# CloudEngineHub/FairyGen

Hardware: AMD Instinct MI355X
Metric: decoded frames/sec (sec/clip in config), Wan2.2-TI2V-5B 704x1280x121 @ 5 steps (higher is better)
Workload: dtype bf16

## Files before the change

fairygen_amd/csrc/attention.hip:

```cpp
#include "common.h"
#include <math.h>
#include <queue>
#include <type_traits>
#include <vector>

#include "attn_w4_asm.inc"
#include "attn_w4p_asm.inc"
#ifndef FG_ATTN_W4
#define FG_ATTN_W4 1
#endif

namespace {

constexpr int kD = 128;
constexpr int kBN = 64;
constexpr int kTileBytes = kBN * kD * 2;
constexpr float kDeferLog2 = 6.0f;

typedef __attribute__((address_space(3))) s16x4 lds_s16x4;

__device__ __forceinline__ int k_lds_off(int row, int chunk) { return row * 256 + ((chunk ^ (row & 15)) << 4); }
__device__ __forceinline__ int v_lds_off(int row, int chunk) {
    return 2048 * (row >> 3) + 512 * (chunk >> 2) + 64 * (row & 7) + 16 * ((chunk & 3) ^ ((row >> 2) & 3));
}

__device__ __forceinline__ float fast_exp2(float x) { return __builtin_amdgcn_exp2f(x); }
__device__ __forceinline__ float max3(float a, float b, float c) {
    float r;
    asm("v_max3_f32 %0, %1, %2, %3" : "=v"(r) : "v"(a), "v"(b), "v"(c));
    return r;
}

__device__ __forceinline__ uint32_t cvt_pk_bf16(float lo, float hi) {
    uint32_t r;
    asm("v_cvt_pk_bf16_f32 %0, %1, %2" : "=v"(r) : "v"(lo), "v"(hi));
    return r;
}

template <int I, int N, typename F>
__device__ __forceinline__ void static_for(F&& f) {
    if constexpr (I < N) {
        f(std::integral_constant<int, I>{});
        static_for<I + 1, N>(f);
    }
}
#ifndef FG_EXP_QK
#define FG_EXP_QK 21
#endif
#ifndef FG_KDIST
#define FG_KDIST 3
#endif
#ifndef FG_VDIST
#define FG_VDIST 2
#endif
__host__ __device__ constexpr int exps_before(int g) {
    return g < 16 ? (FG_EXP_QK * g) / 16 : (FG_EXP_QK + (g - 16) < 32 ? FG_EXP_QK + (g - 16) : 32);
}
static_assert(exps_before(27) == 32, "the last exponential must be issued by gap 26 (its pack feeds the MFMA of gap 28)");

__device__ __forceinline__ float add_f32(float a, float b) {
    float r;
    asm("v_add_f32 %0, %1, %2" : "=v"(r) : "v"(a), "v"(b));
    return r;
}

__device__ __forceinline__ float pair_max(float x) {
    auto r = __builtin_amdgcn_permlane32_swap(__float_as_uint(x), __float_as_uint(x), false, false);
    return fmaxf(__uint_as_float(r[0]), __uint_as_float(r[1]));
}
__device__ __forceinline__ float pair_sum(float x) {
    auto r = __builtin_amdgcn_permlane32_swap(__float_as_uint(x), __float_as_uint(x), false, false);
    return __uint_as_float(r[0]) + __uint_as_float(r[1]);
}

#ifndef FG_ATTN_SCHED
#define FG_ATTN_SCHED 1
#endif
#ifndef FG_ATTN_VARIANT
#define FG_ATTN_VARIANT 8
#endif
#if FG_ATTN_VARIANT == 4
constexpr int kBM = 128;
#else
constexpr int kBM = 256;
#endif

struct AttnParams {
    const bf16* q; const bf16* k; const bf16* v; bf16* out;
    int64_t ldq, ldk, ldv, Nq, Nkv;
    int H, nqb, nfull, R, S, total_direct;
    float scale_log2e;
    float* o_part;
    float* ml_part;
};

template <int WAVES, int QB, bool SHORT_KV = false>
__global__ __launch_bounds__(WAVES * 64, QB == 1 ? 2 : 1) void attn_fwd_kernel(const AttnParams P) {
    const bf16* __restrict__ q = P.q; const bf16* __restrict__ k = P.k; const bf16* __restrict__ v = P.v;
    bf16* __restrict__ out = P.out;
    const int64_t ldq = P.ldq, ldk = P.ldk, ldv = P.ldv, Nq = P.Nq, Nkv = P.Nkv;
    const int H = P.H;
    const float scale_log2e = P.scale_log2e;
    static_assert(WAVES * QB * 32 == kBM, "workgroup rows");
    constexpr int THREADS = WAVES * 64;
    constexpr int NST = (kBN * 16) / THREADS;
    constexpr int ST_ROWS = THREADS / 16;
    __shared__ __attribute__((aligned(16))) char smem[4 * kTileBytes];
    char* const k_lds = smem;
    char* const v_lds = smem + 2 * kTileBytes;

    const int nt = (int)((Nkv + kBN - 1) / kBN);
    int qb, bh, t_begin = 0, t_end = nt, piece = -1;
    if ((int)blockIdx.x < P.total_direct) {
        const int bid = blockIdx.x, xcd = bid & 7, slot = bid >> 3;
        const int qd = P.total_direct >> 3, rm = P.total_direct & 7;
        const int logical = (xcd < rm ? xcd * (qd + 1) : rm * (qd + 1) + (xcd - rm) * qd) + slot;
        qb = logical % P.nfull;
        bh = logical / P.nfull;
    } else {
        piece = (int)blockIdx.x - P.total_direct;
        const int sp = piece % P.S, rq = (piece / P.S) % P.R;
        bh = piece / (P.S * P.R);
        qb = P.nfull + rq;
        t_begin = (int)((int64_t)sp * nt / P.S);
        t_end = (int)((int64_t)(sp + 1) * nt / P.S);
    }
    const int b = bh / H, h = bh % H;

    const int tid = threadIdx.x, lane = tid & 63, wave = tid >> 6;
    const int r = lane & 31, hh = lane >> 5;

    const bf16* qp = q + (int64_t)b * Nq * ldq + (int64_t)h * kD;
    const bf16* kp = k + (int64_t)b * Nkv * ldk + (int64_t)h * kD;
    const bf16* vp = v + (int64_t)b * Nkv * ldv + (int64_t)h * kD;
    bf16* op = out + (int64_t)b * Nq * ((int64_t)H * kD) + (int64_t)h * kD;

    int64_t my_q[QB];
    bool q_valid[QB];
    bf16x8 qf[QB][8];
#pragma unroll
    for (int qi = 0; qi < QB; ++qi) {
        my_q[qi] = (int64_t)qb * kBM + (wave * QB + qi) * 32 + r;
        q_valid[qi] = my_q[qi] < Nq;
        if (!q_valid[qi]) my_q[qi] = Nq - 1;
#pragma unroll
        for (int ks = 0; ks < 8; ++ks)
            qf[qi][ks] = *reinterpret_cast<const bf16x8*>(qp + my_q[qi] * ldq + ks * 16 + hh * 8);
    }

    const int st_row = tid >> 4, st_chunk = tid & 15;
    int st_k[NST], st_v[NST];
#pragma unroll
    for (int i = 0; i < NST; ++i) {
        st_k[i] = k_lds_off(st_row + ST_ROWS * i, st_chunk);
// ... 160 lines not shown
        });
        l_run[0] += ps0 + ps1;
        if (!kTail) {
            absorb_max(pair_max(fmaxf(mt, sn[0][1][15])));
        } else if (t + 1 < t_end) {
            if ((int64_t)(t + 2) * kBN > Nkv) mask_tile(sn, t + 1);
            absorb_max(tile_max(sn));
        }
        __syncthreads();
    };

    f32x16 sA[QB][2], sB[QB][2];
    load_k(t_begin);
    load_v(t_begin);
    write_k(0);
    write_v(0);
    load_k(t_begin + 1);
    write_k(1);
    __syncthreads();
    qk_tile(sA, 0);
    if ((int64_t)(t_begin + 1) * kBN > Nkv) mask_tile(sA, t_begin);
    m_run[0] = tile_max(sA);
    __syncthreads();

    const int t_fast = min(t_end - 1, (int)(Nkv / kBN) - 1);
    int t = t_begin;
    for (; t + 1 < t_fast; t += 2) {
        step_sched(sA, sB, t, std::false_type{}, std::integral_constant<int, 0>{});
        step_sched(sB, sA, t + 1, std::false_type{}, std::integral_constant<int, 1>{});
    }
    for (; t < t_end; ++t) {
        step_sched(sA, sB, t, std::true_type{}, std::integral_constant<int, -1>{});
#pragma unroll
        for (int sub = 0; sub < 2; ++sub) sA[0][sub] = sB[0][sub];
    }
#else
    auto step = [&](f32x16 (&sc)[QB][2], f32x16 (&sn)[QB][2], int t) {
        const int cur = (t - t_begin) & 1;
        load_k(t + 2);
        load_v(t + 1);

        qk_tile(sn, cur ^ 1);
        bf16x8 pf[QB][4];
#pragma unroll
        for (int qi = 0; qi < QB; ++qi) {
            float mt = max3(sc[qi][0][0], sc[qi][1][0], sc[qi][0][1]);
            mt = max3(mt, sc[qi][1][1], sc[qi][0][2]);
#pragma unroll
            for (int j = 2; j < 15; ++j) mt = max3(mt, sc[qi][1][j], sc[qi][0][j + 1]);
            mt = pair_max(fmaxf(mt, sc[qi][1][15]));
            const bool grow = (mt - m_run[qi]) * scale_log2e > kDeferLog2;
            if (__builtin_amdgcn_ballot_w64(grow) != 0) {
                const float m_new = fmaxf(m_run[qi], mt);
                const float alpha = fast_exp2((m_run[qi] - m_new) * scale_log2e);
                m_run[qi] = m_new;
                l_run[qi] *= alpha;
#pragma unroll
                for (int i = 0; i < 4; ++i)
#pragma unroll
                    for (int j = 0; j < 16; ++j) o[qi][i][j] *= alpha;
            }
            const float mb = m_run[qi] * scale_log2e;
            float psum = 0.f;
#pragma unroll
            for (int sub = 0; sub < 2; ++sub)
#pragma unroll
                for (int j = 0; j < 16; ++j) {
                    const float p = fast_exp2(sc[qi][sub][j] * scale_log2e - mb);
                    psum += p;
                    pf[qi][sub * 2 + (j >> 3)][j & 7] = (bf16)p;
                }
            l_run[qi] += psum;
        }

        const char* vb = v_lds + cur * kTileBytes;
#pragma unroll
        for (int kk = 0; kk < 4; ++kk) {
#pragma unroll
            for (int db = 0; db < 4; ++db) {
                union { s16x4 h2[2]; bf16x8 f; } a;
                a.h2[0] = __builtin_amdgcn_ds_read_tr16_b64_v4i16((lds_s16x4*)(vb + v_rd0 + 4096 * kk + 512 * db));
                a.h2[1] = __builtin_amdgcn_ds_read_tr16_b64_v4i16((lds_s16x4*)(vb + v_rd1 + 4096 * kk + 512 * db));
#pragma unroll
                for (int qi = 0; qi < QB; ++qi)
                    o[qi][db] = __builtin_amdgcn_mfma_f32_32x32x16_bf16(a.f, pf[qi][kk], o[qi][db], 0, 0, 0);
            }
        }

        write_k(cur);
        write_v(cur ^ 1);
        if ((int64_t)(t + 2) * kBN > Nkv && t + 1 < t_end) mask_tile(sn, t + 1);
        __syncthreads();
    };

    f32x16 sA[QB][2], sB[QB][2];
    load_k(t_begin);
    load_v(t_begin);
    write_k(0);
    write_v(0);
    load_k(t_begin + 1);
    write_k(1);
    __syncthreads();
    qk_tile(sA, 0);
    if ((int64_t)(t_begin + 1) * kBN > Nkv) mask_tile(sA, t_begin);
    __syncthreads();

    int t = t_begin;
    for (; t + 1 < t_end; t += 2) {
        step(sA, sB, t);
        step(sB, sA, t + 1);
    }
    if (t < t_end) step(sA, sB, t);

#endif

#pragma unroll
    for (int qi = 0; qi < QB; ++qi) {
        const float l_tot = pair_sum(l_run[qi]);
        if (piece < 0) {
            const float inv = 1.0f / l_tot;
            if (q_valid[qi]) {
                bf16* orow = op + my_q[qi] * ((int64_t)H * kD);
#pragma unroll
                for (int db = 0; db < 4; ++db)
#pragma unroll
                    for (int g = 0; g < 4; ++g) {
                        bf16x4 w4;
#pragma unroll
                        for (int j = 0; j < 4; ++j) w4[j] = (bf16)(o[qi][db][4 * g + j] * inv);
                        *reinterpret_cast<bf16x4*>(orow + 32 * db + 8 * g + 4 * hh) = w4;
                    }
            }
        } else {
            const int row = (wave * QB + qi) * 32 + r;
            float* orow = P.o_part + ((int64_t)piece * kBM + row) * kD;
#pragma unroll
            for (int db = 0; db < 4; ++db)
#pragma unroll
                for (int g = 0; g < 4; ++g) {
                    f32x4 w4;
#pragma unroll
                    for (int j = 0; j < 4; ++j) w4[j] = o[qi][db][4 * g + j];
                    *reinterpret_cast<f32x4*>(orow + 32 * db + 8 * g + 4 * hh) = w4;
                }
            if (hh == 0) {
                float* ml = P.ml_part + ((int64_t)piece * kBM + row) * 2;
                ml[0] = m_run[qi];
                ml[1] = l_tot;
            }
        }
    }
}

template <bool PRESCALE>
__global__ __launch_bounds__(256, 1) void attn_fwd_w4_kernel(const AttnParams P) {
    const int nt = (int)((P.Nkv + kBN - 1) / kBN);
    int qb, bh, t_begin = 0, t_end = nt, piece = -1;
    if ((int)blockIdx.x < P.total_direct) {
        const int bid = blockIdx.x, xcd = bid & 7, slot = bid >> 3;
        const int qd = P.total_direct >> 3, rm = P.total_direct & 7;
        const int logical = (xcd < rm ? xcd * (qd + 1) : rm * (qd + 1) + (xcd - rm) * qd) + slot;
        qb = logical % P.nfull;
        bh = logical / P.nfull;
    } else {
        piece = (int)blockIdx.x - P.total_direct;
        const int sp = piece % P.S, rq = (piece / P.S) % P.R;
        bh = piece / (P.S * P.R);
        qb = P.nfull + rq;
        t_begin = (int)((int64_t)sp * nt / P.S);
        t_end = (int)((int64_t)(sp + 1) * nt / P.S);
    }
    const int b = bh / P.H, h = bh % P.H;
    const int64_t hd = (int64_t)P.H * kD;
    const bf16* qp = P.q + (int64_t)b * P.Nq * P.ldq + (int64_t)h * kD;
    const bf16* kp = P.k + (int64_t)b * P.Nkv * P.ldk + (int64_t)h * kD;
    const bf16* vp = P.v + (int64_t)b * P.Nkv * P.ldv + (int64_t)h * kD;
    const void* op;
    const void* mlp;
    if (piece < 0) {
        op = P.out + (int64_t)b * P.Nq * hd + (int64_t)h * kD;
        mlp = op;
    } else {
        op = P.o_part + (int64_t)piece * kBM * kD;
        mlp = P.ml_part + (int64_t)piece * kBM * 2;
    }
    auto sgpr = [](uint32_t x) { return (uint32_t)__builtin_amdgcn_readfirstlane(x); };
    auto sptr = [&](const void* p) {
        const uint64_t u = (uint64_t)p;
        return (const void*)(((uint64_t)sgpr((uint32_t)(u >> 32)) << 32) | sgpr((uint32_t)u));
    };
#define FG_ATTN_W4_OPERANDS                                                                                                       \
    "s"(sptr(qp)), "s"(sptr(kp)), "s"(sptr(vp)), "s"(sptr(op)), "s"(sptr(mlp)), "s"(sgpr(threadIdx.x >> 6)),                     \
        "s"(sgpr((uint32_t)t_begin)), "s"(sgpr((uint32_t)t_end)), "s"(sgpr((uint32_t)qb * kBM)), "s"(sgpr(piece < 0 ? 0u : 1u)), \
        "s"(__builtin_amdgcn_kernarg_segment_ptr())
    if constexpr (PRESCALE) asm volatile(FG_ATTN_W4P_ASM : : FG_ATTN_W4_OPERANDS : FG_ATTN_W4P_CLOBBERS);
    else asm volatile(FG_ATTN_W4_ASM : : FG_ATTN_W4_OPERANDS : FG_ATTN_W4_CLOBBERS);
#undef FG_ATTN_W4_OPERANDS
}

static float pow2_scale_log2e(float scale) {
    const double sl = (double)scale * 1.4426950408889634;
    int e = 0;
    const double m = frexp(sl, &e);
    const double p = fabs(m - 0.5) < 0.25 ? ldexp(0.5, e) : ldexp(1.0, e);
    return fabs(sl / p - 1.0) < 1e-6 && e > -100 && e < 100 ? (float)p : 0.f;
}

__global__ __launch_bounds__(256) void attn_combine_kernel(const AttnParams P) {
    const int rows_per_blk = 8, groups = kBM / rows_per_blk;
    const int blk = blockIdx.x / groups, rowgrp = blockIdx.x % groups;
    const int rq = blk % P.R, bh = blk / P.R;
    const int b = bh / P.H, h = bh % P.H;
    const int qb = P.nfull + rq;
    const int lane32 = threadIdx.x & 31, row = rowgrp * rows_per_blk + (threadIdx.x >> 5);
    const int64_t piece0 = ((int64_t)bh * P.R + rq) * P.S;
    const int64_t qrow = (int64_t)qb * kBM + row;
    if (qrow >= P.Nq) return;
    float mmax = -INFINITY;
    for (int sp = 0; sp < P.S; ++sp) mmax = fmaxf(mmax, P.ml_part[((piece0 + sp) * kBM + row) * 2]);
    float denom = 0.f;
    f32x4 acc = {0.f, 0.f, 0.f, 0.f};
    for (int sp = 0; sp < P.S; ++sp) {
        const float* ml = P.ml_part + ((piece0 + sp) * kBM + row) * 2;
        const float w = fast_exp2((ml[0] - mmax) * P.scale_log2e);
        denom += w * ml[1];
        const f32x4 ov = *reinterpret_cast<const f32x4*>(P.o_part + ((piece0 + sp) * kBM + row) * kD + lane32 * 4);
#pragma unroll
        for (int j = 0; j < 4; ++j) acc[j] += w * ov[j];
    }
    const float inv = 1.0f / denom;
    bf16x4 w4;
#pragma unroll
    for (int j = 0; j < 4; ++j) w4[j] = (bf16)(acc[j] * inv);
    *reinterpret_cast<bf16x4*>(P.out + ((int64_t)b * P.Nq + qrow) * ((int64_t)P.H * kD) + (int64_t)h * kD + lane32 * 4) = w4;
}

struct SplitChoice { int R, S; int64_t ws_bytes; double makespan; };

static double simulate_makespan(int64_t n_direct, int64_t n_pieces, double piece_cost, int cus) {
    const int64_t full = n_direct / cus, rem = n_direct % cus;
    if (n_pieces == 0) return (double)(full + (rem ? 1 : 0));
    std::priority_queue<double, std::vector<double>, std::greater<double>> free_at;
    for (int i = 0; i < cus; ++i) free_at.push((double)(full + (i < rem ? 1 : 0)));
    double last = (double)(full + (rem ? 1 : 0));
    for (int64_t i = 0; i < n_pieces; ++i) {
        const double t = free_at.top() + piece_cost;
        free_at.pop();
        free_at.push(t);
        last = t > last ? t : last;
    }
    return last;
}

static SplitChoice choose_split_uncached(int B, int64_t Nq, int64_t Nkv, int H, int cus, int64_t ws_limit) {
    const int64_t nqb = (Nq + kBM - 1) / kBM, bh = (int64_t)B * H;
    const int nt = (int)((Nkv + kBN - 1) / kBN);
    const int64_t per_piece = (int64_t)kBM * kD * 4 + (int64_t)kBM * 2 * 4;
    SplitChoice best{0, 1, 0, simulate_makespan(bh * nqb, 0, 0.0, cus)};
    const double base = best.makespan;
    const int s_list[] = {2, 3, 4, 5, 6, 8, 12, 16};
    for (int mode = 0; mode < 2; ++mode) {
        const int64_t R = mode == 0 ? 1 : nqb;
        if (mode == 0 && nqb < 2) continue;
        if (mode == 1 && bh * nqb > 4 * (int64_t)cus) continue;
        for (int S : s_list) {
            if (S * 8 > nt) break;
            const int64_t pieces = bh * R * S;
            const int64_t ws = pieces * per_piece;
            if (ws > ws_limit) continue;
            const double cost = 1.0 / S + 3.0 / nt + 0.004;
            const double ms = simulate_makespan(bh * (nqb - R), pieces, cost, cus);
            if (ms < best.makespan) best = SplitChoice{(int)R, S, ws, ms};
        }
    }
    if (best.makespan > 0.98 * base) best = SplitChoice{0, 1, 0, base};
    return best;
}

static SplitChoice choose_split(int B, int64_t Nq, int64_t Nkv, int H, int cus, int64_t ws_limit) {
    struct Key { int B, H, cus; int64_t Nq, Nkv, ws; SplitChoice val; };
    static thread_local Key memo[8];
    static thread_local int next = 0, filled = 0;
    for (int i = 0; i < filled; ++i) {
        const Key& e = memo[i];
        if (e.B == B && e.H == H && e.cus == cus && e.Nq == Nq && e.Nkv == Nkv && e.ws == ws_limit) return e.val;
    }
    const SplitChoice val = choose_split_uncached(B, Nq, Nkv, H, cus, ws_limit);
    memo[next] = Key{B, H, cus, Nq, Nkv, ws_limit, val};
    next = (next + 1) % 8;
    if (filled < 8) ++filled;
    return val;
}

static int device_cus() {
    static thread_local int cached_dev = -1, cached_cus = 256;
    int dev = 0;
    if (hipGetDevice(&dev) != hipSuccess) return 256;
    if (dev != cached_dev) {
        int n = 0;
        if (hipDeviceGetAttribute(&n, hipDeviceAttributeMultiprocessorCount, dev) == hipSuccess && n > 0) cached_cus = n;
        cached_dev = dev;
    }
    return cached_cus * (256 / kBM);
}

}

extern "C" int64_t fg_attn_workspace_bytes(int B, int64_t Nq, int64_t Nkv, int H) {
    if (B <= 0 || Nq <= 0 || Nkv <= 0 || H <= 0) return 0;
    return choose_split(B, Nq, Nkv, H, device_cus(), (int64_t)1 << 40).ws_bytes;
}

extern "C" int fg_attn_split_choice(int B, int64_t Nq, int64_t Nkv, int H, int64_t workspace_bytes, int* R, int* S) {
    FG_CHECK_ARG(B > 0 && Nq > 0 && Nkv > 0 && H > 0 && R && S, "fg_attn_split_choice: bad arguments");
    const SplitChoice sc = choose_split(B, Nq, Nkv, H, device_cus(), workspace_bytes);
    *R = sc.R;
    *S = sc.S;
    return FG_OK;
}

extern "C" int fg_attn_fwd_bf16(const void* q, int64_t ldq, const void* k, int64_t ldk, const void* v, int64_t ldv,
                                void* out, int B, int64_t Nq, int64_t Nkv, int H, int D, float scale, void* workspace,
                                int64_t workspace_bytes, fg_stream_t stream) {
    FG_CHECK_ARG(q && k && v && out, "fg_attn_fwd_bf16: null pointer");
    FG_CHECK_ARG(D == kD, "fg_attn_fwd_bf16: only head_dim 128 is supported (got %d)", D);
    FG_CHECK_ARG(B > 0 && H > 0 && Nq > 0 && Nkv > 0, "fg_attn_fwd_bf16: B, H, Nq, Nkv must be positive");
    FG_CHECK_ARG(scale > 0.f, "fg_attn_fwd_bf16: scale must be positive");
    const int64_t hd = (int64_t)H * D;
    FG_CHECK_ARG(ldq >= hd && ldk >= hd && ldv >= hd && ldq % 8 == 0 && ldk % 8 == 0 && ldv % 8 == 0,
                 "fg_attn_fwd_bf16: leading dimensions must be >= H*D and multiples of 8");
    FG_CHECK_ARG(FG_ALIGNED16(q) && FG_ALIGNED16(k) && FG_ALIGNED16(v) && FG_ALIGNED16(out) && FG_ALIGNED16(workspace),
                 "fg_attn_fwd_bf16: pointers must be 16-byte aligned");
    FG_CHECK_ARG(workspace_bytes >= 0 && (workspace != nullptr || workspace_bytes == 0), "fg_attn_fwd_bf16: bad workspace");
    const int64_t nqb = (Nq + kBM - 1) / kBM;
    FG_CHECK_ARG((Nkv + 6 * kBN) * ldk * 2 < (1ll << 32) && (Nkv + 6 * kBN) * ldv * 2 < (1ll << 32),
                 "fg_attn_fwd_bf16: K/V of one batch element must span < 4 GiB (32-bit buffer offsets)");
    FG_CHECK_ARG(Nq * ldq * 2 < (1ll << 32) && Nq * hd * 2 < (1ll << 32),
                 "fg_attn_fwd_bf16: Q / O of one batch element must span < 4 GiB (32-bit buffer offsets)");
    const SplitChoice sc = choose_split(B, Nq, Nkv, H, device_cus(), workspace_bytes);
    AttnParams P;
    P.q = (const bf16*)q; P.k = (const bf16*)k; P.v = (const bf16*)v; P.out = (bf16*)out;
    P.ldq = ldq; P.ldk = ldk; P.ldv = ldv; P.Nq = Nq; P.Nkv = Nkv; P.H = H;
    P.nqb = (int)nqb; P.R = sc.R; P.S = sc.S; P.nfull = (int)(nqb - sc.R);
    const int64_t total_direct = (int64_t)B * H * P.nfull, pieces = (int64_t)B * H * sc.R * sc.S;
    FG_CHECK_ARG(total_direct + pieces < (1ll << 30), "fg_attn_fwd_bf16: grid too large");
    P.total_direct = (int)total_direct;
    P.scale_log2e = scale * 1.4426950408889634f;
    P.o_part = (float*)workspace;
    P.ml_part = (float*)workspace + pieces * kBM * kD;
#if FG_ATTN_VARIANT == 4
    hipLaunchKernelGGL((attn_fwd_kernel<4, 1>), dim3((unsigned)(total_direct + pieces)), dim3(256), 0, (hipStream_t)stream, P);
#else
#if FG_ATTN_W4
    static const bool use_w4 = [] { const char* e = getenv("FAIRYGEN_ATTN_W4"); return e ? atoi(e) != 0 : true; }();
    if (Nkv > 1024 && use_w4) {
        static const hipError_t attr0 = hipFuncSetAttribute(reinterpret_cast<const void*>(attn_fwd_w4_kernel<false>),
                                                            hipFuncAttributeMaxDynamicSharedMemorySize, 8 * kTileBytes);
        static const hipError_t attr1 = hipFuncSetAttribute(reinterpret_cast<const void*>(attn_fwd_w4_kernel<true>),
                                                            hipFuncAttributeMaxDynamicSharedMemorySize, 8 * kTileBytes);
        FG_CHECK_ARG(attr0 == hipSuccess && attr1 == hipSuccess, "fg_attn_fwd_bf16: cannot reserve 128 KiB of LDS: %s",
                     hipGetErrorString(attr0 == hipSuccess ? attr1 : attr0));
        const float p2 = pow2_scale_log2e(scale);
        if (p2 > 0.f) {
            P.scale_log2e = p2;
            hipLaunchKernelGGL(attn_fwd_w4_kernel<true>, dim3((unsigned)(total_direct + pieces)), dim3(256), 8 * kTileBytes, (hipStream_t)stream, P);
        } else {
            hipLaunchKernelGGL(attn_fwd_w4_kernel<false>, dim3((unsigned)(total_direct + pieces)), dim3(256), 8 * kTileBytes, (hipStream_t)stream, P);
        }
    } else
#endif
    if (Nkv <= 1024)
        hipLaunchKernelGGL((attn_fwd_kernel<8, 1, true>), dim3((unsigned)(total_direct + pieces)), dim3(512), 0, (hipStream_t)stream, P);
    else
        hipLaunchKernelGGL((attn_fwd_kernel<8, 1, false>), dim3((unsigned)(total_direct + pieces)), dim3(512), 0, (hipStream_t)stream, P);
#endif
    if (int e = fg_launch_status("fg_attn_fwd_bf16")) return e;
    if (pieces > 0) {
        hipLaunchKernelGGL(attn_combine_kernel, dim3((unsigned)((int64_t)B * H * sc.R * (kBM / 8))), dim3(256), 0, (hipStream_t)stream, P);
        return fg_launch_status("fg_attn_fwd_bf16 (combine)");
    }
    return FG_OK;
}
```

fairygen_amd/hip.py:

```python
import ctypes
import os

import torch

_LIB_PATH = os.environ.get("FAIRYGEN_HIP_LIB") or os.path.join(os.path.dirname(os.path.abspath(__file__)), "libfairygen_hip.so")
_lib = None

ABI_VERSION = 5

_i64, _i32, _f32, _vp = ctypes.c_int64, ctypes.c_int, ctypes.c_float, ctypes.c_void_p

_SIGNATURES = {
    "fg_ln_modulate_bf16": [_vp, _vp, _vp, _vp, _i64, _i32, _f32, _i64, _i64, _i64, _vp],
    "fg_ln_affine_bf16": [_vp, _vp, _vp, _vp, _i64, _i32, _f32, _vp],
    "fg_ln_modulate_fp8_bf16": [_vp, _vp, _vp, _vp, _vp, _i64, _i32, _f32, _i64, _i64, _i64, _f32, _vp],
    "fg_residual_ln_fp8_bf16": [_vp, _vp, _vp, _vp, _vp, _vp, _vp, _vp, _i32, _i64, _i32, _f32, _i64, _i64, _i64, _f32, _vp],
    "fg_ln_modulate_dual_bf16": [_vp, _vp, _vp, _vp, _vp, _vp, _i64, _i32, _f32, _i64, _i64, _i64, _f32, _vp],
    "fg_ln_affine_dual_bf16": [_vp, _vp, _vp, _vp, _vp, _vp, _i64, _i32, _f32, _f32, _vp],
    "fg_gate_residual_bf16": [_vp, _vp, _vp, _vp, _i64, _i32, _i64, _i64, _i64, _vp],
    "fg_residual_ln_bf16": [_vp, _vp, _vp, _vp, _vp, _vp, _vp, _i32, _i64, _i32, _f32, _i64, _i64, _i64, _vp],
    "fg_rmsnorm_rope_bf16": [_vp, _i64, _vp, _vp, _vp, _i32, _vp, _i64, _i32, _i32, _f32, _vp],
    "fg_rmsnorm_rope_grouped_bf16": [_vp, _i64, _vp, _vp, _vp, _i32, _vp, _i64, _i32, _i32, _f32, _i32, _i64, _i64, _vp],
    "fg_copy_groups_bf16": [_vp, _i64, _i64, _vp, _i64, _i64, _i32, _i64, _i32, _vp],
    "fg_fp8_quant_rows_bf16": [_vp, _i64, _vp, _vp, _vp, _i64, _i32, _i32, _f32, _vp],
    "fg_act_bf16": [_vp, _vp, _i64, _i32, _vp],
    "fg_gemm_epilogue_bf16": [_vp, _i64, _vp, _vp, _vp, _i64, _i64, _i64, _i64, _i32, _vp, _i64, _i64, _i64, _vp, _vp],
    "fg_gemm_fp8_bf16": [_vp, _i64, _vp, _vp, _vp, _vp, _i64, _i64, _i64, _i64, _i32, _vp, _i64, _i64, _i64, _vp, _vp],
    "fg_lora_apply_bf16": [_vp, _i64, _vp, _vp, _vp, _i64, _i64, _i64, _i64, _i64, _i64, _i32, _vp, _i64, _i64, _i64, _vp],
    "fg_attn_fwd_bf16": [_vp, _i64, _vp, _i64, _vp, _i64, _vp, _i32, _i64, _i64, _i32, _i32, _f32, _vp, _i64, _vp],
    "fg_cfg_euler_bf16": [_vp, _vp, _vp, _vp, _i64, _f32, _f32, _vp],
    "fg_vae_rmsnorm_silu_bf16": [_vp, _vp, _vp, _i64, _i32, _i32, _vp],
    "fg_conv_pack_weight_bf16": [_vp, _vp, _i32, _i32, _i32, _i32, _i32, _vp],
    "fg_conv3d_cl_bf16": [_vp, _vp, _vp, _vp, _vp, _i32, _i32, _i32, _i32, _i32, _i32, _i32, _i32, _i32, _vp],
    "fg_dupup3d_add_bf16": [_vp, _vp, _vp, _i32, _i32, _i32, _i32, _i32, _i32, _i32, _i32, _vp],
    "fg_softmax_rows_f32_bf16": [_vp, _vp, _i64, _i64, _f32, _vp],
    "fg_vae_latent_to_cl_bf16": [_vp, _vp, _vp, _vp, _i32, _i32, _i32, _i32, _vp],
    "fg_vae_unpatchify_bf16": [_vp, _vp, _i32, _i32, _i32, _i32, _i32, _i32, _vp],
    "fg_vae_tile_accumulate_bf16": [_vp, _vp, _vp, _i32, _i32, _i32, _i32, _i32, _i32, _i32, _i32, _i32, _i32, _i32, _vp],
    "fg_vae_tile_finalize_bf16": [_vp, _vp, _i32, _i32, _i32, _i32, _i32, _vp],
    "fg_vae_patchify_bf16": [_vp, _vp, _i32, _i32, _i32, _vp],
    "fg_avgdown3d_add_bf16": [_vp, _vp, _vp, _i32, _i32, _i32, _i32, _i32, _i32, _i32, _vp],
    "fg_vae_latent_from_cl_bf16": [_vp, _vp, _vp, _vp, _i32, _i32, _i32, _i32, _i32, _vp],
    "fg_video_to_uint8": [_vp, _vp, _i32, _i32, _i32, _vp],
    "fg_softmax_bias_bf16": [_vp, _vp, _vp, _vp, _i64, _i64, _vp],
    "fg_gated_gelu_bf16": [_vp, _vp, _vp, _i64, _vp],
}
EXPORTED_SYMBOLS = sorted(list(_SIGNATURES) + ["fg_version", "fg_last_error", "fg_conv_packed_bytes", "fg_attn_workspace_bytes", "fg_attn_split_choice",
                                                   "fg_conv_tile_choice", "fg_gemm_workspace_bytes", "fg_gemm_debug_grid"])


class HipLibraryError(RuntimeError):
    pass


def library_path():
    return _LIB_PATH


def load():
    global _lib
    if _lib is not None:
        return _lib
    if not os.path.exists(_LIB_PATH):
        raise HipLibraryError(
            f"{_LIB_PATH} not found: build it with `make -C fairygen_amd/csrc` (or __graft_entry__.build()). "
            "fairygen_amd has no CPU / PyTorch fallback for its kernels.")
    lib = ctypes.CDLL(_LIB_PATH)
    lib.fg_version.restype = ctypes.c_int
    lib.fg_last_error.restype = ctypes.c_char_p
    lib.fg_conv_packed_bytes.restype = ctypes.c_int64
    lib.fg_conv_packed_bytes.argtypes = [_i32] * 5
    lib.fg_attn_workspace_bytes.restype = ctypes.c_int64
    lib.fg_attn_workspace_bytes.argtypes = [_i32, _i64, _i64, _i32]
    lib.fg_conv_tile_choice.restype = ctypes.c_int
    lib.fg_conv_tile_choice.argtypes = [_i32] * 4
    lib.fg_gemm_workspace_bytes.restype = ctypes.c_int64
    lib.fg_gemm_workspace_bytes.argtypes = [_i64] * 3
    lib.fg_gemm_debug_grid.restype = ctypes.c_int
    lib.fg_gemm_debug_grid.argtypes = [_i32]
    lib.fg_attn_split_choice.restype = ctypes.c_int
    lib.fg_attn_split_choice.argtypes = [_i32, _i64, _i64, _i32, _i64, ctypes.POINTER(ctypes.c_int), ctypes.POINTER(ctypes.c_int)]
    for name, argtypes in _SIGNATURES.items():
        fn = getattr(lib, name)
        fn.restype = ctypes.c_int
        fn.argtypes = argtypes
    if lib.fg_version() != ABI_VERSION:
        raise HipLibraryError(f"ABI mismatch: library {lib.fg_version()} != binding {ABI_VERSION}")
    _lib = lib
    return lib


def _call(name, *args):
    lib = load()
    rc = getattr(lib, name)(*args)
    if rc != 0:
        raise HipLibraryError(f"{name} failed ({rc}): {lib.fg_last_error().decode()}")


def _stream(t):
    return ctypes.c_void_p(torch.cuda.current_stream(t.device).cuda_stream)


def _dev(t, name, dtype=torch.bfloat16):
    if not isinstance(t, torch.Tensor) or t.device.type != "cuda":
        raise HipLibraryError(f"{name}: expected a tensor on a HIP device, got {getattr(t, 'device', type(t))} "
                              "(no CPU fallback)")
    if t.dtype != dtype:
        raise HipLibraryError(f"{name}: expected dtype {dtype}, got {t.dtype}")
    return t


def _ptr(t):
    return ctypes.c_void_p(t.data_ptr()) if t is not None else ctypes.c_void_p(0)


def _rows(t, name):
    _dev(t, name)
    if not t.is_contiguous():
        raise HipLibraryError(f"{name}: must be contiguous")
    return t.numel() // t.shape[-1], t.shape[-1]


class ModTable:

    def __init__(self, table, first_rows=0):
        _dev(table, "mod table")
        assert table.dim() == 3 and table.is_contiguous()
        self.table, self.first_rows = table, int(first_rows)
        self.mod_rows, self.k, self.c = table.shape
        self.ld = self.k * self.c

    def vec(self, j):
        return ctypes.c_void_p(self.table.data_ptr() + 2 * j * self.c)


def _mod_args(mod, rows):
    if mod.mod_rows not in (1, 2, rows):
        raise HipLibraryError(f"modulation table has {mod.mod_rows} rows; expected 1, 2 or {rows}")
    return mod.mod_rows, mod.first_rows, mod.ld


def ln_modulate(x, mod, shift_idx, scale_idx, eps, out=None):
    rows, c = _rows(x, "x")
    out = torch.empty_like(x) if out is None else out
    _call("fg_ln_modulate_bf16", _ptr(x), mod.vec(shift_idx), mod.vec(scale_idx), _ptr(out), rows, c, eps,
          *_mod_args(mod, rows), _stream(x))
    return out


def ln_affine(x, w, b, eps, out=None):
    rows, c = _rows(x, "x")
    _dev(w, "w"), _dev(b, "b")
    out = torch.empty_like(x) if out is None else out
    _call("fg_ln_affine_bf16", _ptr(x), _ptr(w), _ptr(b), _ptr(out), rows, c, eps, _stream(x))
    return out


def gate_residual(x, y, mod=None, gate_idx=None, out=None):
    rows, c = _rows(x, "x")
    _rows(y, "y")
    out = torch.empty_like(x) if out is None else out
    if mod is None:
        _call("fg_gate_residual_bf16", _ptr(x), _ptr(y), None, _ptr(out), rows, c, 1, 0, 0, _stream(x))
    else:
        _call("fg_gate_residual_bf16", _ptr(x), _ptr(y), mod.vec(gate_idx), _ptr(out), rows, c,
              *_mod_args(mod, rows), _stream(x))
    return out


def residual_ln_modulate(x, y, mod, gate_idx, shift_idx, scale_idx, eps, x_out=None, norm_out=None, norm_mod=None):
    rows, c = _rows(x, "x")
    _rows(y, "y")
    norm_mod = mod if norm_mod is None else norm_mod
    if (norm_mod.mod_rows, norm_mod.first_rows, norm_mod.ld) != (mod.mod_rows, mod.first_rows, mod.ld):
        raise HipLibraryError("residual_ln_modulate: gate and norm tables must share rows / first_rows / ld")
    x_out = torch.empty_like(x) if x_out is None else x_out
    norm_out = torch.empty_like(x) if norm_out is None else norm_out
    gate = mod.vec(gate_idx) if gate_idx is not None else None
    _call("fg_residual_ln_bf16", _ptr(x), _ptr(y), gate, _ptr(x_out), norm_mod.vec(shift_idx),
          norm_mod.vec(scale_idx), _ptr(norm_out), 0, rows, c, eps, *_mod_args(mod, rows), _stream(x))
    return x_out, norm_out


def residual_ln_affine(x, y, w, b, eps, mod=None, gate_idx=None, x_out=None, norm_out=None):
    rows, c = _rows(x, "x")
    _rows(y, "y")
    _dev(w, "w"), _dev(b, "b")
    x_out = torch.empty_like(x) if x_out is None else x_out
    norm_out = torch.empty_like(x) if norm_out is None else norm_out
    if mod is None:
        gate, margs = None, (1, 0, 0)
    else:
        gate, margs = mod.vec(gate_idx), _mod_args(mod, rows)
    _call("fg_residual_ln_bf16", _ptr(x), _ptr(y), gate, _ptr(x_out), _ptr(w), _ptr(b), _ptr(norm_out), 1, rows, c,
          eps, *margs, _stream(x))
    return x_out, norm_out


def _fp8_rows_out(x):
    rows, c = _rows(x, "x")
    return (torch.empty((rows, c), dtype=torch.float8_e4m3fn, device=x.device),
            torch.empty((rows, 1), dtype=torch.float32, device=x.device))


def ln_modulate_fp8(x, mod, shift_idx, scale_idx, eps):
    rows, c = _rows(x, "x")
    q, sc = _fp8_rows_out(x)
    _call("fg_ln_modulate_fp8_bf16", _ptr(x), mod.vec(shift_idx), mod.vec(scale_idx), _ptr(q), _ptr(sc), rows, c, eps,
          *_mod_args(mod, rows), FP8_E4M3FN_MAX, _stream(x))
    return q, sc


def ln_modulate_dual(x, mod, shift_idx, scale_idx, eps, out=None):
    rows, c = _rows(x, "x")
    out = torch.empty_like(x) if out is None else _dev(out, "out")
    q, sc = _fp8_rows_out(x)
    _call("fg_ln_modulate_dual_bf16", _ptr(x), mod.vec(shift_idx), mod.vec(scale_idx), _ptr(out), _ptr(q), _ptr(sc), rows, c, eps,
          *_mod_args(mod, rows), FP8_E4M3FN_MAX, _stream(x))
    return out, (q, sc)


def ln_affine_dual(x, w, b, eps, out=None):
    rows, c = _rows(x, "x")
    _dev(w, "w"), _dev(b, "b")
    out = torch.empty_like(x) if out is None else _dev(out, "out")
    q, sc = _fp8_rows_out(x)
    _call("fg_ln_affine_dual_bf16", _ptr(x), _ptr(w), _ptr(b), _ptr(out), _ptr(q), _ptr(sc), rows, c, eps, FP8_E4M3FN_MAX, _stream(x))
    return out, (q, sc)


def residual_ln_modulate_fp8(x, y, mod, gate_idx, shift_idx, scale_idx, eps, x_out=None, norm_mod=None):
    rows, c = _rows(x, "x")
# ... 397 lines not shown
```

include/fairygen_hip.h:

```cpp
#ifndef FAIRYGEN_HIP_H
#define FAIRYGEN_HIP_H

#include <stdint.h>

#ifdef __cplusplus
extern "C" {
#endif

#define FG_OK        0
#define FG_EINVAL   (-1)
#define FG_ELAUNCH  (-2)

typedef void* fg_stream_t;

int         fg_version(void);
const char* fg_last_error(void);


int fg_ln_modulate_bf16(const void* x, const void* shift, const void* scale, void* out,
                        int64_t rows, int C, float eps,
                        int64_t mod_rows, int64_t first_rows, int64_t mod_ld, fg_stream_t stream);

int fg_ln_affine_bf16(const void* x, const void* w, const void* b, void* out,
                      int64_t rows, int C, float eps, fg_stream_t stream);

int fg_gate_residual_bf16(const void* x, const void* y, const void* gate, void* out,
                          int64_t rows, int C,
                          int64_t mod_rows, int64_t first_rows, int64_t mod_ld, fg_stream_t stream);

int fg_residual_ln_bf16(const void* x, const void* y, const void* gate, void* x_out,
                        const void* p0, const void* p1, void* norm_out, int mode,
                        int64_t rows, int C, float eps,
                        int64_t mod_rows, int64_t first_rows, int64_t mod_ld, fg_stream_t stream);

int fg_ln_modulate_fp8_bf16(const void* x, const void* shift, const void* scale, void* out_fp8, float* out_scale,
                            int64_t rows, int C, float eps, int64_t mod_rows, int64_t first_rows, int64_t mod_ld,
                            float fp8_max, fg_stream_t stream);
int fg_residual_ln_fp8_bf16(const void* x, const void* y, const void* gate, void* x_out, const void* p0, const void* p1,
                            void* norm_fp8, float* norm_scale, int mode, int64_t rows, int C, float eps,
                            int64_t mod_rows, int64_t first_rows, int64_t mod_ld, float fp8_max, fg_stream_t stream);

int fg_ln_modulate_dual_bf16(const void* x, const void* shift, const void* scale, void* out, void* out_fp8, float* out_scale,
                             int64_t rows, int C, float eps, int64_t mod_rows, int64_t first_rows, int64_t mod_ld,
                             float fp8_max, fg_stream_t stream);
int fg_ln_affine_dual_bf16(const void* x, const void* w, const void* b, void* out, void* out_fp8, float* out_scale,
                           int64_t rows, int C, float eps, float fp8_max, fg_stream_t stream);

int64_t fg_gemm_workspace_bytes(int64_t M, int64_t N, int64_t K);
int fg_gemm_epilogue_bf16(const void* a, int64_t lda, const void* w, const void* bias, void* c, int64_t ldc,
                          int64_t M, int64_t N, int64_t K, int mode, const void* gate, int64_t gate_rows, int64_t gate_ld,
                          int64_t first_rows, void* workspace, fg_stream_t stream);

int fg_lora_apply_bf16(const void* x, int64_t ldx, const void* a, const void* b, void* out, int64_t ldc, int64_t M, int64_t K,
                       int64_t Ng, int64_t R, int64_t G, int mode, const void* gate, int64_t gate_rows, int64_t gate_ld,
                       int64_t first_rows, fg_stream_t stream);

int fg_gemm_debug_grid(int workgroups);

int fg_gemm_fp8_bf16(const void* a_fp8, int64_t lda, const float* scale_a, const void* w_fp8, const void* bias, void* c, int64_t ldc,
                     int64_t M, int64_t N, int64_t K, int mode, const void* gate, int64_t gate_rows, int64_t gate_ld,
                     int64_t first_rows, void* workspace, fg_stream_t stream);

int fg_rmsnorm_rope_bf16(const void* x, int64_t ldx, const void* weight,
                         const void* cos_tab, const void* sin_tab, int table_f32, void* out,
                         int64_t rows, int C, int num_heads, float eps, fg_stream_t stream);

int fg_rmsnorm_rope_grouped_bf16(const void* x, int64_t ldx, const void* weight,
                                 const void* cos_tab, const void* sin_tab, int table_f32, void* out,
                                 int64_t rows, int C, int num_heads, float eps,
                                 int group_cols, int64_t out_group_stride, int64_t out_ld, fg_stream_t stream);

int fg_copy_groups_bf16(const void* src, int64_t src_group_stride, int64_t src_ld,
                        void* dst, int64_t dst_group_stride, int64_t dst_ld,
                        int groups, int64_t rows, int cols, fg_stream_t stream);

int fg_fp8_quant_rows_bf16(const void* x, int64_t ldx, void* out_fp8, float* scale, void* act_out,
                           int64_t rows, int C, int act, float fp8_max, fg_stream_t stream);

int fg_act_bf16(const void* x, void* out, int64_t n, int kind, fg_stream_t stream);

int64_t fg_attn_workspace_bytes(int B, int64_t Nq, int64_t Nkv, int H);
int fg_attn_split_choice(int B, int64_t Nq, int64_t Nkv, int H, int64_t workspace_bytes, int* R, int* S);
int fg_attn_fwd_bf16(const void* q, int64_t ldq, const void* k, int64_t ldk, const void* v, int64_t ldv,
                     void* out, int B, int64_t Nq, int64_t Nkv, int H, int D, float scale,
                     void* workspace, int64_t workspace_bytes, fg_stream_t stream);

int fg_cfg_euler_bf16(const void* latents, const void* posi, const void* nega, void* out,
                      int64_t n, float cfg_scale, float dsigma, fg_stream_t stream);


int fg_vae_rmsnorm_silu_bf16(const void* x, const void* gamma, void* out,
                             int64_t pixels, int C, int apply_silu, fg_stream_t stream);

int64_t fg_conv_packed_bytes(int Cout, int Cin, int kt, int kh, int kw);
int fg_conv_pack_weight_bf16(const void* w, void* packed, int Cout, int Cin, int kt, int kh, int kw,
                             fg_stream_t stream);

int fg_conv3d_cl_bf16(const void* x, const void* w_packed, const void* bias,
                      const void* residual, void* out,
                      int T, int H, int W, int Cin, int Cout, int kt, int ks,
                      int resample, int time_interleave, fg_stream_t stream);
int fg_conv_tile_choice(int T, int H, int W, int Cout);

int fg_dupup3d_add_bf16(const void* x, const void* main_path, void* out,
                        int T, int H, int W, int Cin, int Cout, int ft, int fs, int first_chunk,
                        fg_stream_t stream);

int fg_softmax_rows_f32_bf16(const float* scores, void* probs, int64_t rows, int64_t cols, float scale,
                             fg_stream_t stream);

int fg_vae_latent_to_cl_bf16(const void* z, const void* mean, const void* inv_std, void* out,
                             int C, int T, int H, int W, fg_stream_t stream);

int fg_vae_unpatchify_bf16(const void* x, void* video, int T, int H, int W, int F, int t0, int do_clamp,
                           fg_stream_t stream);

int fg_vae_tile_accumulate_bf16(const void* tile, void* values, void* weight,
                                int C, int F, int Hv, int Wv, int th, int tw, int y0, int x0,
                                int border_h, int border_w, int bound_bits, fg_stream_t stream);

int fg_vae_tile_finalize_bf16(void* values, const void* weight, int C, int F, int Hv, int Wv, int do_clamp,
                              fg_stream_t stream);

int fg_vae_patchify_bf16(const void* video, void* out, int T, int H, int W, fg_stream_t stream);

int fg_avgdown3d_add_bf16(const void* x, const void* main_path, void* out,
                          int T, int H, int W, int Cin, int Cout, int ft, int fs, fg_stream_t stream);

int fg_vae_latent_from_cl_bf16(const void* x, const void* mean, const void* inv_std, void* out,
                               int Z, int Cx, int T, int H, int W, fg_stream_t stream);

int fg_video_to_uint8(const void* video, void* out_u8, int F, int H, int W, fg_stream_t stream);


int fg_softmax_bias_bf16(const void* scores, const void* bias, const int* key_mask, void* probs,
                         int64_t rows, int64_t cols, fg_stream_t stream);

int fg_gated_gelu_bf16(const void* fc1, const void* gate, void* out, int64_t n, fg_stream_t stream);

#ifdef __cplusplus
}
#endif
#endif
```

Before: 15.32.

## Add persistent cross-attention kernel for 512-token keys with LDS-resident K

Adds a dedicated 512-thread attention kernel for the case where the key/value length is exactly 512, as in text cross-attention. It loads all eight K tiles into LDS once per workgroup and keeps them there. It then loops persistently over several query blocks, streaming V through a double buffer and prefetching the next Q block. The aim is to cut repeated K loads, split-KV workspace traffic and launch imbalance for the short-key cross-attention calls. It is enabled by default with a runtime toggle. In exchange it reserves 160 KiB of LDS, carries a large register footprint, and assumes Nkv exactly equals 512.

```diff
diff --git a/fairygen_amd/csrc/attention.hip b/fairygen_amd/csrc/attention.hip
--- a/fairygen_amd/csrc/attention.hip
+++ b/fairygen_amd/csrc/attention.hip
@@ -1,5 +1,6 @@
 #include "common.h"
 #include <math.h>
+#include <atomic>
 #include <queue>
 #include <type_traits>
 #include <vector>
@@ -466,6 +467,238 @@
     }
 }
 
+constexpr int kXTiles = 8;
+constexpr int kXLdsBytes = (2 + kXTiles) * kTileBytes;
+
+__global__ __launch_bounds__(512, 2) void attn_cross512_kernel(const AttnParams P, const int n_wg, const int nbh) {
+    const bf16* __restrict__ q = P.q; const bf16* __restrict__ k = P.k; const bf16* __restrict__ v = P.v;
+    bf16* __restrict__ out = P.out;
+    const int64_t ldq = P.ldq, ldk = P.ldk, ldv = P.ldv, Nq = P.Nq;
+    const int H = P.H;
+    const float scale_log2e = P.scale_log2e;
+    constexpr int NST = 2, ST_ROWS = 32;
+    extern __shared__ __attribute__((aligned(16))) char smem[];
+    char* const v_lds = smem;
+    char* const k_lds = smem + 2 * kTileBytes;
+
+    int bh, qb, qstride;
+    {
+        const int bid = blockIdx.x, xcd = bid & 7, slot = bid >> 3;
+        const int qd = n_wg >> 3, rm = n_wg & 7;
+        const int logical = (xcd < rm ? xcd * (qd + 1) : rm * (qd + 1) + (xcd - rm) * qd) + slot;
+        const int base = n_wg / nbh, rem = n_wg % nbh;
+        if (logical < rem * (base + 1)) {
+            bh = logical / (base + 1); qb = logical % (base + 1); qstride = base + 1;
+        } else {
+            const int l2 = logical - rem * (base + 1);
+            bh = rem + l2 / base; qb = l2 % base; qstride = base;
+        }
+    }
+    const int b = bh / H, h = bh % H;
+
+    const int tid = threadIdx.x, lane = tid & 63, wave = tid >> 6;
+    const int r = lane & 31, hh = lane >> 5;
+
+    const bf16* qp = q + (int64_t)b * Nq * ldq + (int64_t)h * kD;
+    const bf16* kp = k + (int64_t)b * (kXTiles * kBN) * ldk + (int64_t)h * kD;
+    const bf16* vp = v + (int64_t)b * (kXTiles * kBN) * ldv + (int64_t)h * kD;
+    bf16* op = out + (int64_t)b * Nq * ((int64_t)H * kD) + (int64_t)h * kD;
+
+    const int st_row = tid >> 4, st_chunk = tid & 15;
+    {
+        u32x4 kr[kXTiles * NST];
+#pragma unroll
+        for (int i = 0; i < kXTiles * NST; ++i)
+            kr[i] = *reinterpret_cast<const u32x4*>(kp + (int64_t)(st_row + ST_ROWS * i) * ldk + st_chunk * 8);
+#pragma unroll
+        for (int i = 0; i < kXTiles * NST; ++i)
+            *reinterpret_cast<u32x4*>(k_lds + (i >> 1) * kTileBytes + k_lds_off(st_row + ST_ROWS * (i & 1), st_chunk)) = kr[i];
+    }
+
+    int st_v[NST];
+#pragma unroll
+    for (int i = 0; i < NST; ++i) st_v[i] = v_lds_off(st_row + ST_ROWS * i, st_chunk);
+    const uint32_t v_bytes = (uint32_t)((kXTiles * kBN - 1) * ldv * 2 + kD * 2);
+    const __amdgpu_buffer_rsrc_t v_rsrc = __builtin_amdgcn_make_buffer_rsrc(const_cast<bf16*>(vp), 0, v_bytes, 0x00020000);
+    const uint32_t v_tile_stride = (uint32_t)(kBN * ldv * 2);
+    uint32_t v_off[NST];
+#pragma unroll
+    for (int i = 0; i < NST; ++i) v_off[i] = (uint32_t)((st_row + ST_ROWS * i) * ldv * 2 + st_chunk * 16);
+    u32x4 vreg[NST];
+    auto load_v = [&](int t) {
+        const uint32_t base = (uint32_t)t * v_tile_stride;
+#pragma unroll
+        for (int i = 0; i < NST; ++i) vreg[i] = __builtin_amdgcn_raw_buffer_load_b128(v_rsrc, v_off[i] + base, 0, 0);
+    };
+    auto write_v = [&](int buf) {
+#pragma unroll
+        for (int i = 0; i < NST; ++i) *reinterpret_cast<u32x4*>(v_lds + buf * kTileBytes + st_v[i]) = vreg[i];
+    };
+
+    auto load_q = [&](int blk, bf16x8 (&dst)[8], int64_t& row, bool& valid) {
+        row = (int64_t)blk * kBM + wave * 32 + r;
+        valid = row < Nq;
+        if (!valid) row = Nq - 1;
+#pragma unroll
+        for (int ks = 0; ks < 8; ++ks) dst[ks] = *reinterpret_cast<const bf16x8*>(qp + row * ldq + ks * 16 + hh * 8);
+    };
+
+    bf16x8 qf[8], qfn[8];
+    int64_t my_q, my_qn;
+    bool q_valid, q_validn;
+
+    int k_rd[8];
+#pragma unroll
+    for (int ks = 0; ks < 8; ++ks) k_rd[ks] = k_lds_off(r, 2 * ks + hh);
+    const int tr_g1 = (lane >> 4) & 1, tr_q = (lane & 15) >> 2, tr_p = lane & 3;
+    const int v_rd0 = v_lds_off(4 * hh + tr_q, 2 * tr_g1 + (tr_p >> 1)) + 8 * (tr_p & 1);
+    const int v_rd1 = v_lds_off(8 + 4 * hh + tr_q, 2 * tr_g1 + (tr_p >> 1)) + 8 * (tr_p & 1);
+
+    f32x16 o[4];
+    float m_run, l_run = 0.f;
+#pragma unroll
+    for (int i = 0; i < 4; ++i)
+#pragma unroll
+        for (int j = 0; j < 16; ++j) o[i][j] = 0.f;
+
+    auto absorb_max = [&](float mt) {
+        const bool grow = (mt - m_run) * scale_log2e > kDeferLog2;
+        if (__builtin_amdgcn_ballot_w64(grow) != 0) {
+            const float m_new = fmaxf(m_run, mt);
+            const float alpha = fast_exp2((m_run - m_new) * scale_log2e);
+            m_run = m_new;
+            l_run *= alpha;
+#pragma unroll
+            for (int i = 0; i < 4; ++i)
+#pragma unroll
+                for (int j = 0; j < 16; ++j) o[i][j] *= alpha;
+        }
+    };
+
+    auto step = [&](f32x16 (&sc)[2], f32x16 (&sn)[2], const bf16x8 (&qq)[8], int t, auto new_tag, auto pre_tag, auto cur_tag) -> float {
+        constexpr bool kNew = decltype(new_tag)::value;
+        constexpr bool kPre = decltype(pre_tag)::value;
+        constexpr int cur = decltype(cur_tag)::value;
+        const char* kb = k_lds + ((t + 1) & (kXTiles - 1)) * kTileBytes;
+        const char* vb = v_lds + cur * kTileBytes;
+        load_v((t + 1) & (kXTiles - 1));
+        const float mb = m_run * scale_log2e;
+        float ps0 = 0.f, ps1 = 0.f, mt = 0.f;
+        float pe[32];
+        union PF { uint32_t w[4]; bf16x8 f; } pf[4];
+        bf16x8 ka[16];
+        union VF { s16x4 h2[2]; bf16x8 f; } va[16];
+        auto read_k = [&](int g) { ka[g] = *reinterpret_cast<const bf16x8*>(kb + k_rd[g & 7] + (g >> 3) * 8192); };
+        auto read_v = [&](int p) {
+            va[p].h2[0] = __builtin_amdgcn_ds_read_tr16_b64_v4i16((lds_s16x4*)(vb + v_rd0 + 4096 * (p >> 2) + 512 * (p & 3)));
+            va[p].h2[1] = __builtin_amdgcn_ds_read_tr16_b64_v4i16((lds_s16x4*)(vb + v_rd1 + 4096 * (p >> 2) + 512 * (p & 3)));
+        };
+        auto do_exp = [&](int e) {
+            const float p = fast_exp2(sc[e >> 4][e & 15] * scale_log2e - mb);
+            pe[e] = p;
+        };
+        auto do_add = [&](int e) { if (e & 1) ps1 = add_f32(ps1, pe[e]); else ps0 = add_f32(ps0, pe[e]); };
+        auto do_pack = [&](int u) { pf[u >> 2].w[u & 3] = cvt_pk_bf16(pe[2 * u], pe[2 * u + 1]); };
+
+        static_for<0, FG_KDIST>([&](auto i) { read_k(decltype(i)::value); });
+        __builtin_amdgcn_sched_barrier(0);
+        static_for<0, 32>([&](auto gc) {
+            constexpr int g = decltype(gc)::value;
+            constexpr int e0 = exps_before(g), e1 = exps_before(g + 1), ep = g == 0 ? 0 : exps_before(g - 1);
+            if constexpr (g < 16) {
+                constexpr int sub = g >> 3, ks = g & 7;
+                if constexpr (ks == 0) {
+#pragma unroll
+                    for (int j = 0; j < 16; ++j) sn[sub][j] = 0.f;
+                }
+                sn[sub] = __builtin_amdgcn_mfma_f32_32x32x16_bf16(ka[g], qq[ks], sn[sub], 0, 0, 0);
+                if constexpr (g + FG_KDIST < 16) read_k(g + FG_KDIST);
+                if constexpr (kPre && g >= 8) qfn[ks] = *reinterpret_cast<const bf16x8*>(qp + my_qn * ldq + ks * 16 + hh * 8);
+            } else {
+                constexpr int p = g - 16;
+                o[p & 3] = __builtin_amdgcn_mfma_f32_32x32x16_bf16(va[p].f, pf[p >> 2].f, o[p & 3], 0, 0, 0);
+            }
+            if constexpr (g + FG_VDIST >= 16 && g + FG_VDIST < 32) read_v(g + FG_VDIST - 16);
+            constexpr int u0 = ep / 2, u1 = e0 / 2;
+            if constexpr (u1 > u0) do_pack(u0);
+            if constexpr (u1 > u0 + 1) do_pack(u0 + 1);
+            if constexpr (e1 > e0) do_exp(e0);
+            if constexpr (e1 > e0 + 1) do_exp(e0 + 1);
+            if constexpr (e0 > ep) do_add(ep);
+            if constexpr (e0 > ep + 1) do_add(ep + 1);
+            if constexpr (g >= 17) {
+                constexpr int i = g - 17;
+                if constexpr (i == 0) mt = max3(sn[0][0], sn[1][0], sn[0][1]);
+                else mt = max3(mt, sn[1][i], sn[0][i + 1]);
+            }
+            if constexpr (g == 30) write_v(cur ^ 1);
+            __builtin_amdgcn_sched_barrier(0);
+        });
+        l_run += ps0 + ps1;
+        mt = pair_max(fmaxf(mt, sn[1][15]));
+        if constexpr (!kNew) absorb_max(mt);
+        __syncthreads();
+        return mt;
+    };
+
+    f32x16 sA[2], sB[2];
+    load_q(qb, qf, my_q, q_valid);
+    load_v(0);
+    write_v(0);
+    __syncthreads();
+#pragma unroll
+    for (int sub = 0; sub < 2; ++sub) {
+#pragma unroll
+        for (int j = 0; j < 16; ++j) sA[sub][j] = 0.f;
+#pragma unroll
+        for (int ks = 0; ks < 8; ++ks) {
+            const bf16x8 a = *reinterpret_cast<const bf16x8*>(k_lds + k_rd[ks] + sub * 8192);
+            sA[sub] = __builtin_amdgcn_mfma_f32_32x32x16_bf16(a, qf[ks], sA[sub], 0, 0, 0);
+        }
+    }
+    float m0 = fmaxf(sA[0][0], sA[1][0]);
+#pragma unroll
+    for (int j = 1; j < 16; ++j) m0 = fmaxf(m0, fmaxf(sA[0][j], sA[1][j]));
+    m_run = pair_max(m0);
+
+    for (; qb < P.nqb; qb += qstride) {
+        my_qn = (int64_t)(qb + qstride < P.nqb ? qb + qstride : qb) * kBM + wave * 32 + r;
+        q_validn = my_qn < Nq;
+        if (!q_validn) my_qn = Nq - 1;
+        for (int t = 0; t < 6; t += 2) {
+            step(sA, sB, qf, t, std::false_type{}, std::false_type{}, std::integral_constant<int, 0>{});
+            step(sB, sA, qf, t + 1, std::false_type{}, std::false_type{}, std::integral_constant<int, 1>{});
+        }
+        step(sA, sB, qf, 6, std::false_type{}, std::true_type{}, std::integral_constant<int, 0>{});
+        const float m_next = step(sB, sA, qfn, 7, std::true_type{}, std::false_type{}, std::integral_constant<int, 1>{});
+
+        const float l_tot = pair_sum(l_run);
+        const float inv = 1.0f / l_tot;
+        if (q_valid) {
+            bf16* orow = op + my_q * ((int64_t)H * kD);
+#pragma unroll
+            for (int db = 0; db < 4; ++db)
+#pragma unroll
+                for (int g = 0; g < 4; ++g) {
+                    bf16x4 w4;
+#pragma unroll
+                    for (int j = 0; j < 4; ++j) w4[j] = (bf16)(o[db][4 * g + j] * inv);
+                    *reinterpret_cast<bf16x4*>(orow + 32 * db + 8 * g + 4 * hh) = w4;
+                }
+        }
+#pragma unroll
+        for (int i = 0; i < 4; ++i)
+#pragma unroll
+            for (int j = 0; j < 16; ++j) o[i][j] = 0.f;
+        l_run = 0.f;
+        m_run = m_next;
+#pragma unroll
+        for (int ks = 0; ks < 8; ++ks) qf[ks] = qfn[ks];
+        my_q = my_qn;
+        q_valid = q_validn;
+    }
+}
+
 template <bool PRESCALE>
 __global__ __launch_bounds__(256, 1) void attn_fwd_w4_kernel(const AttnParams P) {
     const int nt = (int)((P.Nkv + kBN - 1) / kBN);
@@ -606,6 +839,8 @@
     return val;
 }
 
+static std::atomic<int> g_cross512{1};
+
 static int device_cus() {
     static thread_local int cached_dev = -1, cached_cus = 256;
     int dev = 0;
@@ -619,6 +854,8 @@
 }
 
 }
+
+extern "C" int fg_attn_cross512_enable(int enable) { return g_cross512.exchange(enable != 0 ? 1 : 0); }
 
 extern "C" int64_t fg_attn_workspace_bytes(int B, int64_t Nq, int64_t Nkv, int H) {
     if (B <= 0 || Nq <= 0 || Nkv <= 0 || H <= 0) return 0;
@@ -665,6 +902,15 @@
 #if FG_ATTN_VARIANT == 4
     hipLaunchKernelGGL((attn_fwd_kernel<4, 1>), dim3((unsigned)(total_direct + pieces)), dim3(256), 0, (hipStream_t)stream, P);
 #else
+    if (Nkv == kXTiles * kBN && g_cross512.load(std::memory_order_relaxed)) {
+        static const hipError_t attr = hipFuncSetAttribute(reinterpret_cast<const void*>(attn_cross512_kernel),
+                                                           hipFuncAttributeMaxDynamicSharedMemorySize, kXLdsBytes);
+        FG_CHECK_ARG(attr == hipSuccess, "fg_attn_fwd_bf16: cannot reserve 160 KiB of LDS: %s", hipGetErrorString(attr));
+        const int64_t nbh = (int64_t)B * H, cus = device_cus();
+        const int64_t n_wg = nbh >= cus ? nbh : (nbh * nqb < cus ? nbh * nqb : cus);
+        hipLaunchKernelGGL(attn_cross512_kernel, dim3((unsigned)n_wg), dim3(512), kXLdsBytes, (hipStream_t)stream, P, (int)n_wg, (int)nbh);
+        return fg_launch_status("fg_attn_fwd_bf16 (cross512)");
+    }
 #if FG_ATTN_W4
     static const bool use_w4 = [] { const char* e = getenv("FAIRYGEN_ATTN_W4"); return e ? atoi(e) != 0 : true; }();
     if (Nkv > 1024 && use_w4) {
diff --git a/fairygen_amd/hip.py b/fairygen_amd/hip.py
--- a/fairygen_amd/hip.py
+++ b/fairygen_amd/hip.py
@@ -45,7 +45,7 @@
     "fg_softmax_bias_bf16": [_vp, _vp, _vp, _vp, _i64, _i64, _vp],
     "fg_gated_gelu_bf16": [_vp, _vp, _vp, _i64, _vp],
 }
-EXPORTED_SYMBOLS = sorted(list(_SIGNATURES) + ["fg_version", "fg_last_error", "fg_conv_packed_bytes", "fg_attn_workspace_bytes", "fg_attn_split_choice",
+EXPORTED_SYMBOLS = sorted(list(_SIGNATURES) + ["fg_version", "fg_last_error", "fg_conv_packed_bytes", "fg_attn_workspace_bytes", "fg_attn_split_choice", "fg_attn_cross512_enable",
                                                    "fg_conv_tile_choice", "fg_gemm_workspace_bytes", "fg_gemm_debug_grid"])
 
 
@@ -78,6 +78,8 @@
     lib.fg_gemm_workspace_bytes.argtypes = [_i64] * 3
     lib.fg_gemm_debug_grid.restype = ctypes.c_int
     lib.fg_gemm_debug_grid.argtypes = [_i32]
+    lib.fg_attn_cross512_enable.restype = ctypes.c_int
+    lib.fg_attn_cross512_enable.argtypes = [_i32]
     lib.fg_attn_split_choice.restype = ctypes.c_int
     lib.fg_attn_split_choice.argtypes = [_i32, _i64, _i64, _i32, _i64, ctypes.POINTER(ctypes.c_int), ctypes.POINTER(ctypes.c_int)]
     for name, argtypes in _SIGNATURES.items():
diff --git a/include/fairygen_hip.h b/include/fairygen_hip.h
--- a/include/fairygen_hip.h
+++ b/include/fairygen_hip.h
@@ -84,6 +84,7 @@
 int fg_attn_fwd_bf16(const void* q, int64_t ldq, const void* k, int64_t ldk, const void* v, int64_t ldv,
                      void* out, int B, int64_t Nq, int64_t Nkv, int H, int D, float scale,
                      void* workspace, int64_t workspace_bytes, fg_stream_t stream);
+int fg_attn_cross512_enable(int enable);
 
 int fg_cfg_euler_bf16(const void* latents, const void* posi, const void* nega, void* out,
                       int64_t n, float cfg_scale, float dsigma, fg_stream_t stream);
```

Result: no change. 15.32, median of 2 (+0.0%).
